# dmosopt/dmosopt

Hardware: NVIDIA H100
Metric: candidate-evals/sec (GP+sort+HV) pop=65536 dim=30 obj=3 (higher is better)
Workload: dtype f64 results; GP variance contraction in split-fp16 wgmma with fp32 accumulation (precision=auto: calibrated against the float64 path, 0 of 65535 rows of the last step recomputed in float64); ranks on u32 ids

## Files before the change

dmosopt_b200/_lib.py:

```python

import ctypes
import os
import threading

import numpy as np

_HERE = os.path.dirname(os.path.abspath(__file__))
LIB_PATH = os.path.join(_HERE, "libdmosopt_b200.so")

METRIC_NONE, METRIC_CROWDING, METRIC_EUCLIDEAN = 0, 1, 2
KERNEL_MATERN52, KERNEL_RBF = 0, 1
GP_FP64, GP_TENSOR, GP_AUTO = 0, 1, 2
HV_MAX_OBJECTIVES = 8

_c_i64 = ctypes.c_int64
_c_u64 = ctypes.c_uint64
_c_int = ctypes.c_int
_c_dbl = ctypes.c_double
_vp = ctypes.c_void_p

_SIGNATURES = {
    "dmo_version": (_c_int, []),
    "dmo_create": (_c_int, [_c_int, ctypes.POINTER(_vp)]),
    "dmo_destroy": (_c_int, [_vp]),
    "dmo_last_error": (ctypes.c_char_p, [_vp]),
    "dmo_synchronize": (_c_int, [_vp]),
    "dmo_stream": (_vp, [_vp]),
    "dmo_launch_count": (_c_i64, [_vp]),
    "dmo_sm_count": (_c_int, [_vp]),
    "dmo_timer_begin": (_c_int, [_vp]),
    "dmo_timer_end": (_c_int, [_vp, ctypes.POINTER(ctypes.c_float)]),
    "dmo_host_alloc": (_c_int, [ctypes.POINTER(_vp), _c_u64]),
    "dmo_host_free": (_c_int, [_vp]),
    "dmo_device_alloc": (_c_int, [_vp, ctypes.POINTER(_vp), _c_u64]),
    "dmo_device_free": (_c_int, [_vp, _vp]),
    "dmo_memcpy": (_c_int, [_vp, _vp, _vp, _c_u64]),
    "dmo_flush_l2": (_c_int, [_vp]),
    "dmo_transfer_bytes": (_c_int, [_vp, ctypes.POINTER(_c_u64), ctypes.POINTER(_c_u64)]),
    "dmo_profile_enable": (_c_int, [_vp, _c_int]),
    "dmo_profile_report": (_c_int, [_vp, ctypes.c_char_p, _c_u64]),
    "dmo_round_f32": (_c_int, [_vp, _vp, _c_i64]),
    "dmo_rank_nd": (_c_int, [_vp, _vp, _c_i64, _c_int, _vp]),
    "dmo_crowding_distance": (_c_int, [_vp, _vp, _c_i64, _c_int, _vp]),
    "dmo_euclidean_distance": (_c_int, [_vp, _vp, _c_i64, _c_int, _vp]),
    "dmo_order_mo": (_c_int, [_vp, _vp, _c_i64, _c_int, _c_int, _vp, _c_int, _vp, _vp, _vp]),
    "dmo_remove_worst": (_c_int, [_vp, _vp, _vp, _c_i64, _c_int, _c_int, _c_int, _vp, _c_int, _c_i64, _vp, _vp, _vp, _vp]),
    "dmo_remove_worst_pair": (_c_int, [_vp, _vp, _vp, _c_i64, _vp, _vp, _c_i64, _c_int, _c_int, _c_int, _c_i64, _vp, _vp, _vp, _vp]),
    "dmo_tournament": (_c_int, [_vp, _vp, _vp, _c_i64, _c_i64, _c_u64, _c_u64, _vp, _vp]),
    "dmo_mutation_u": (_c_int, [_vp, _vp, _vp, _c_i64, _c_int, _vp, _vp, _vp, _c_dbl, _vp]),
    "dmo_sbx_u": (_c_int, [_vp, _vp, _vp, _vp, _c_i64, _c_int, _vp, _vp, _vp, _vp, _vp]),
    "dmo_nsga2_plan_length": (_c_i64, [_c_i64, _c_dbl, _c_dbl]),
    "dmo_nsga2_generate": (
        _c_int,
        [_vp, _vp, _c_i64, _c_int, _vp, _c_i64, _c_i64, _c_dbl, _c_dbl, _c_dbl, _vp, _vp, _vp, _vp, _c_u64, _c_u64, _vp, _vp, _vp, _vp],
    ),
    "dmo_gp_create": (_c_int, [_vp, _c_i64, _c_int, _c_int, _c_int, _vp, _vp, _vp, _c_int, _vp, _vp, _vp, _vp, _vp, _vp, _vp, ctypes.POINTER(_vp)]),
    "dmo_gp_destroy": (_c_int, [_vp, _vp]),
    "dmo_gp_fit": (_c_int, [_vp, _c_i64, _c_int, _c_int, _c_int, _vp, _vp, _vp, _vp, _vp, _c_dbl, _vp, _vp, _vp]),
    "dmo_gp_set_linear_mean": (_c_int, [_vp, _vp, _vp, _vp]),
    "dmo_gp_predict": (_c_int, [_vp, _vp, _vp, _c_i64, _vp, _vp, _c_int]),
    "dmo_gp_auto_info": (_c_int, [_vp, _vp, ctypes.POINTER(_c_int), ctypes.POINTER(_c_int), ctypes.POINTER(_c_dbl), ctypes.POINTER(_c_dbl),
                                  ctypes.POINTER(_c_dbl), ctypes.POINTER(_c_i64)]),
    "dmo_gp_covariance_groups": (_c_int, [_vp, _vp, ctypes.POINTER(_c_int), _vp]),
    "dmo_mtgp_create": (_c_int, [_vp, _c_i64, _c_int, _c_int, _vp, _vp, _vp, _vp, _vp, _vp, _vp, _vp, _vp, _vp, _vp, ctypes.POINTER(_c_dbl),
                                 ctypes.POINTER(_vp)]),
    "dmo_mtgp_predict": (_c_int, [_vp, _vp, _vp, _c_i64, _vp, _vp, _c_int]),
    "dmo_mtgp_destroy": (_c_int, [_vp, _vp]),
    "dmo_svgp_create": (_c_int, [_vp, _c_int, _c_int, _c_i64, _c_int, _vp, _vp, _vp, _vp, _vp, _vp, _c_dbl, _vp, _vp, _vp, _vp, _vp,
                                 ctypes.POINTER(_vp)]),
    "dmo_svgp_predict": (_c_int, [_vp, _vp, _vp, _c_i64, _vp, _vp, _c_int]),
    "dmo_svgp_groups": (_c_int, [_vp, _vp, ctypes.POINTER(_c_int), ctypes.POINTER(_c_int)]),
    "dmo_svgp_destroy": (_c_int, [_vp, _vp]),
    "dmo_svgp_optimal_q": (_c_int, [_vp, _c_i64, _c_i64, _c_int, _c_int, _vp, _vp, _vp, _vp, _vp, _vp, _c_dbl, _c_int, _vp, _vp]),
    "dmo_mtgp_lml_grad": (_c_int, [_vp, _c_i64, _c_int, _c_int, _vp, _vp, _vp, _vp, _vp, _vp, _vp, _vp, _vp, _vp, _vp, _vp, _vp]),
    "dmo_gp_lml_grad": (_c_int, [_vp, _c_i64, _c_int, _c_int, _vp, _vp, _vp, _vp, _vp, _vp, _vp, _vp, _vp, _vp, _vp, _vp, _vp]),
    "dmo_nsga2_step": (_c_int, [_vp, _vp, _vp, _vp, _vp, _c_i64, _c_int, _c_int, _c_dbl, _c_dbl, _c_dbl, _vp, _vp, _vp, _vp, _c_u64, _c_u64,
                                _c_int, _c_int, _c_int, _c_int, _vp, _vp, _vp]),
    "dmo_hypervolume": (_c_int, [_vp, _vp, _c_i64, _c_int, _vp, ctypes.POINTER(_c_dbl)]),
    "dmo_hypervolume_ranked": (_c_int, [_vp, _vp, _c_i64, _c_int, _vp, _vp, ctypes.POINTER(_c_dbl)]),
    "dmo_ehvi_select": (_c_int, [_vp, _vp, _c_i64, _vp, _vp, _c_i64, _c_int, _vp, _c_int, _c_i64, _vp, _vp]),
    "dmo_get_duplicates": (_c_int, [_vp, _vp, _c_i64, _c_int, _c_dbl, _vp]),
    "dmo_get_duplicates_pair": (_c_int, [_vp, _vp, _c_i64, _vp, _c_i64, _c_int, _c_dbl, _vp]),
    "dmo_age_survival": (_c_int, [_vp, _vp, _vp, _c_i64, _c_int, _c_dbl, _vp, _c_int, _vp]),
    "dmo_smpso_velocity": (_c_int, [_vp, _vp, _vp, _vp, _vp, _c_int, _c_i64, _c_int, _c_dbl, _c_dbl, _c_dbl, _c_dbl, _c_dbl, _c_dbl, _vp, _vp, _vp]),
    "dmo_mutate_groups": (_c_int, [_vp, _vp, _c_i64, _c_i64, _c_i64, _c_int, _vp, _vp, _vp, _c_dbl, _c_u64, _c_u64, _vp, _vp]),
    "dmo_cmaes_sample": (_c_int, [_vp, _vp, _vp, _c_int, _vp, _c_i64, _vp, _vp, _c_i64, _c_int, _vp]),
    "dmo_cmaes_update_cholesky": (_c_int, [_vp, _vp, _vp, _vp, _vp, _vp, _c_i64, _c_int, _c_dbl, _c_dbl, _c_dbl]),
    "dmo_gather_rows": (_c_int, [_vp, _vp, _vp, _vp, _vp, _c_i64, _c_i64, _vp]),
    "dmo_cmaes_generate": (_c_int, [_vp, _vp, _vp, _c_int, _vp, _c_i64, _vp, _vp, _c_i64, _c_int, _vp, _vp, _vp]),
    "dmo_cmaes_step_z": (_c_int, [_vp, _vp, _vp, _vp, _vp, _vp, _vp, _vp, _c_i64, _c_int, _vp]),
    "dmo_scale_rows": (_c_int, [_vp, _vp, _c_i64, _c_i64, _vp, _vp, _vp, _c_i64]),
    "dmo_benchmark_eval": (_c_int, [_vp, _c_int, _vp, _c_i64, _c_int, _c_int, _c_dbl, _vp]),
    "dmo_smpso_generate": (_c_int, [_vp, _vp, _vp, _c_int, _c_i64, _c_int, _vp, _vp, _vp, _c_dbl, _c_u64, _c_u64, _vp, _vp]),
    "dmo_smpso_update": (_c_int, [_vp, _vp, _vp, _vp, _vp, _c_int, _vp, _c_int, _c_i64, _c_int, _c_int, _c_int, _vp, _vp, _vp, _vp, _vp, _vp, _vp]),
}

_lib = None
_ctx = None
_ctx_device = None
_lock = threading.Lock()


class DmoError(RuntimeError):
    pass


def load_library(path=None):
    global _lib
    if _lib is not None:
        return _lib
    path = path or LIB_PATH
    if not os.path.exists(path):
        raise DmoError(
            f"dmosopt_b200: CUDA library {path} not found. Build it with `python -m dmosopt_b200.build` "
            "(nvcc, sm_90a). There is no CPU fallback."
        )
# ... 46 lines not shown
    with _lock:
        while len(_worker_ctx) <= i:
            h = _vp()
            st = load_library().dmo_create(_ctx_device, ctypes.byref(h))
            if st != 0 or not h.value:
                raise DmoError(f"dmosopt_b200: dmo_create(device={_ctx_device}) failed for a worker context (status {st})")
            _worker_ctx.append(h)
    assert main is not None
    return _worker_ctx[i]


def worker_pool():
    global _worker_pool
    if _worker_pool is None:
        from concurrent.futures import ThreadPoolExecutor

        _worker_pool = ThreadPoolExecutor(max_workers=8, thread_name_prefix="dmosopt_b200_worker")
    return _worker_pool


def _ptr(a):
    if a is None:
        return None
    if isinstance(a, np.ndarray):
        return a.ctypes.data
    if hasattr(a, "data_ptr"):
        return int(a.data_ptr())
    if isinstance(a, int):
        return a
    raise TypeError(f"cannot pass {type(a)} to the CUDA library")


def _f64(a):
    return np.ascontiguousarray(a, dtype=np.float64)


def synchronize():
    _check(load_library().dmo_synchronize(context()), "dmo_synchronize")


def stream_ptr():
    return int(load_library().dmo_stream(context()))


def launch_count():
    lib = load_library()
    return int(lib.dmo_launch_count(context())) + sum(int(lib.dmo_launch_count(c)) for c in _worker_ctx)


def sm_count():
    return int(load_library().dmo_sm_count(context()))


def timer_begin():
    _check(load_library().dmo_timer_begin(context()), "dmo_timer_begin")


def timer_end():
    ms = ctypes.c_float()
    _check(load_library().dmo_timer_end(context(), ctypes.byref(ms)), "dmo_timer_end")
    return float(ms.value)


def flush_l2():
    _check(load_library().dmo_flush_l2(context()), "dmo_flush_l2")


def transfer_bytes():
    h2d = d2h = 0
    for c in [context()] + list(_worker_ctx):
        a, b = _c_u64(0), _c_u64(0)
        _check(load_library().dmo_transfer_bytes(c, ctypes.byref(a), ctypes.byref(b)), "dmo_transfer_bytes")
        h2d, d2h = h2d + int(a.value), d2h + int(b.value)
    return h2d, d2h


def profile_enable(on=True):
    _check(load_library().dmo_profile_enable(context(), 1 if on else 0), "dmo_profile_enable")


def profile_report():
    buf = ctypes.create_string_buffer(1 << 16)
    _check(load_library().dmo_profile_report(context(), buf, len(buf)), "dmo_profile_report")
    out = {}
    for line in buf.value.decode().splitlines():
        name, ms, cnt = line.rsplit(" ", 2)
        out[name] = (float(ms), int(cnt))
    return out


def round_f32(dev_ptr, n):
    _check(load_library().dmo_round_f32(context(), _ptr(dev_ptr), int(n)), "dmo_round_f32")


class DeviceArray:

    def __init__(self, shape, dtype=np.float64):
        self.shape = tuple(np.atleast_1d(shape).tolist()) if not isinstance(shape, tuple) else shape
        self.dtype = np.dtype(dtype)
        self.nbytes = int(np.prod(self.shape)) * self.dtype.itemsize
        p = _vp()
        _check(load_library().dmo_device_alloc(context(), ctypes.byref(p), max(self.nbytes, 1)), "dmo_device_alloc")
        self.ptr = p.value

    def data_ptr(self):
        return self.ptr
# ... 893 lines not shown
```

dmosopt_b200/csrc/gp_tensor.cu:

```cuda
#include <cuda.h>
#include <cuda_fp16.h>
#include <cudaTypedefs.h>
#include <stdlib.h>

#include "gp.cuh"

namespace {

constexpr int TN = 256;
constexpr int TMV = 128;
constexpr int TK = 32;
constexpr int UK = 16;
constexpr int STAGES = 4;
constexpr int A_BYTES = TMV * TK * 2;
constexpr int B_BYTES = TN * TK * 2;
constexpr int STAGE_BYTES = 2 * A_BYTES + 2 * B_BYTES;
constexpr size_t GEMM_SMEM = (size_t)STAGES * STAGE_BYTES + 1024 + 256;
constexpr int NTHREADS = 384;

__device__ __forceinline__ uint32_t smem_u32(const void* p) { return (uint32_t)__cvta_generic_to_shared(p); }

__device__ __forceinline__ void mbar_init(uint64_t* bar, uint32_t count) {
  asm volatile("mbarrier.init.shared::cta.b64 [%0], %1;" ::"r"(smem_u32(bar)), "r"(count) : "memory");
}
__device__ __forceinline__ void mbar_arrive(uint64_t* bar) {
  asm volatile("mbarrier.arrive.shared::cta.b64 _, [%0];" ::"r"(smem_u32(bar)) : "memory");
}
__device__ __forceinline__ void mbar_expect_tx(uint64_t* bar, uint32_t bytes) {
  asm volatile("mbarrier.arrive.expect_tx.shared::cta.b64 _, [%0], %1;" ::"r"(smem_u32(bar)), "r"(bytes) : "memory");
}
__device__ __forceinline__ bool mbar_try_wait(uint64_t* bar, uint32_t parity) {
  uint32_t ok;
  asm volatile(
      "{\n"
      ".reg .pred p;\n"
      "mbarrier.try_wait.parity.shared::cta.b64 p, [%1], %2;\n"
      "selp.u32 %0, 1, 0, p;\n"
      "}\n"
      : "=r"(ok)
      : "r"(smem_u32(bar)), "r"(parity)
      : "memory");
  return ok != 0;
}
__device__ __forceinline__ void mbar_wait(uint64_t* bar, uint32_t parity, volatile int* abort_flag) {
  uint32_t spins = 0;
  while (!mbar_try_wait(bar, parity)) {
    if ((++spins & 0x3FFu) == 0u) {
      if (*abort_flag) return;
      if (spins > (1u << 22)) {
        *abort_flag = 1;
        return;
      }
    }
  }
}

__device__ __forceinline__ void tma_load_2d(const CUtensorMap* map, uint64_t* bar, void* dst, int c0, int c1) {
  asm volatile(
      "cp.async.bulk.tensor.2d.shared::cluster.global.tile.mbarrier::complete_tx::bytes [%0], [%1, {%3, %4}], [%2];" ::"r"(
          smem_u32(dst)),
      "l"(map), "r"(smem_u32(bar)), "r"(c0), "r"(c1)
      : "memory");
}

__device__ __forceinline__ uint64_t make_sdesc64(uint32_t smem_addr) {
  return (uint64_t)((smem_addr >> 4) & 0x3FFFu) | (1ull << 16) | ((uint64_t)(512 >> 4) << 32) | (2ull << 62);
}

__device__ __forceinline__ void wgmma_fence() { asm volatile("wgmma.fence.sync.aligned;" ::: "memory"); }
__device__ __forceinline__ void wgmma_commit() { asm volatile("wgmma.commit_group.sync.aligned;" ::: "memory"); }
template <int N>
__device__ __forceinline__ void wgmma_wait() {
  asm volatile("wgmma.wait_group.sync.aligned %0;" ::"n"(N) : "memory");
}

__device__ __forceinline__ void wgmma_f16_m64n256(float (&d)[128], uint64_t adesc, uint64_t bdesc, uint32_t accumulate) {
  asm volatile(
      "{\n"
      ".reg .pred p;\n"
      "setp.ne.b32 p, %130, 0;\n"
      "wgmma.mma_async.sync.aligned.m64n256k16.f32.f16.f16 "
      "{"
      "%0, %1, %2, %3, %4, %5, %6, %7, %8, %9, %10, %11, %12, %13, %14, %15, "
      "%16, %17, %18, %19, %20, %21, %22, %23, %24, %25, %26, %27, %28, %29, %30, %31, "
      "%32, %33, %34, %35, %36, %37, %38, %39, %40, %41, %42, %43, %44, %45, %46, %47, "
      "%48, %49, %50, %51, %52, %53, %54, %55, %56, %57, %58, %59, %60, %61, %62, %63, "
      "%64, %65, %66, %67, %68, %69, %70, %71, %72, %73, %74, %75, %76, %77, %78, %79, "
      "%80, %81, %82, %83, %84, %85, %86, %87, %88, %89, %90, %91, %92, %93, %94, %95, "
      "%96, %97, %98, %99, %100, %101, %102, %103, %104, %105, %106, %107, %108, %109, %110, %111, "
      "%112, %113, %114, %115, %116, %117, %118, %119, %120, %121, %122, %123, %124, %125, %126, %127}, "
      "%128, %129, p, 1, 1, 0, 0;\n"
      "}\n"
      : "+f"(d[0]), "+f"(d[1]), "+f"(d[2]), "+f"(d[3]), "+f"(d[4]), "+f"(d[5]), "+f"(d[6]), "+f"(d[7]),
        "+f"(d[8]), "+f"(d[9]), "+f"(d[10]), "+f"(d[11]), "+f"(d[12]), "+f"(d[13]), "+f"(d[14]), "+f"(d[15]),
        "+f"(d[16]), "+f"(d[17]), "+f"(d[18]), "+f"(d[19]), "+f"(d[20]), "+f"(d[21]), "+f"(d[22]), "+f"(d[23]),
        "+f"(d[24]), "+f"(d[25]), "+f"(d[26]), "+f"(d[27]), "+f"(d[28]), "+f"(d[29]), "+f"(d[30]), "+f"(d[31]),
        "+f"(d[32]), "+f"(d[33]), "+f"(d[34]), "+f"(d[35]), "+f"(d[36]), "+f"(d[37]), "+f"(d[38]), "+f"(d[39]),
        "+f"(d[40]), "+f"(d[41]), "+f"(d[42]), "+f"(d[43]), "+f"(d[44]), "+f"(d[45]), "+f"(d[46]), "+f"(d[47]),
        "+f"(d[48]), "+f"(d[49]), "+f"(d[50]), "+f"(d[51]), "+f"(d[52]), "+f"(d[53]), "+f"(d[54]), "+f"(d[55]),
        "+f"(d[56]), "+f"(d[57]), "+f"(d[58]), "+f"(d[59]), "+f"(d[60]), "+f"(d[61]), "+f"(d[62]), "+f"(d[63]),
        "+f"(d[64]), "+f"(d[65]), "+f"(d[66]), "+f"(d[67]), "+f"(d[68]), "+f"(d[69]), "+f"(d[70]), "+f"(d[71]),
        "+f"(d[72]), "+f"(d[73]), "+f"(d[74]), "+f"(d[75]), "+f"(d[76]), "+f"(d[77]), "+f"(d[78]), "+f"(d[79]),
        "+f"(d[80]), "+f"(d[81]), "+f"(d[82]), "+f"(d[83]), "+f"(d[84]), "+f"(d[85]), "+f"(d[86]), "+f"(d[87]),
        "+f"(d[88]), "+f"(d[89]), "+f"(d[90]), "+f"(d[91]), "+f"(d[92]), "+f"(d[93]), "+f"(d[94]), "+f"(d[95]),
        "+f"(d[96]), "+f"(d[97]), "+f"(d[98]), "+f"(d[99]), "+f"(d[100]), "+f"(d[101]), "+f"(d[102]), "+f"(d[103]),
        "+f"(d[104]), "+f"(d[105]), "+f"(d[106]), "+f"(d[107]), "+f"(d[108]), "+f"(d[109]), "+f"(d[110]), "+f"(d[111]),
        "+f"(d[112]), "+f"(d[113]), "+f"(d[114]), "+f"(d[115]), "+f"(d[116]), "+f"(d[117]), "+f"(d[118]), "+f"(d[119]),
        "+f"(d[120]), "+f"(d[121]), "+f"(d[122]), "+f"(d[123]), "+f"(d[124]), "+f"(d[125]), "+f"(d[126]), "+f"(d[127])
      : "l"(adesc), "l"(bdesc), "r"(accumulate)
      : "memory");
}

struct GemmParams {
  int M, n_pb, n_jt, n_q;
  int64_t k_rows, l_rows;
  const float* inv_scale;
  double* vnorm;
  int64_t vn_ld;
  int* abort_flag;
};

__device__ __forceinline__ int item_blocks(const GemmParams& p, int q) { return q == p.n_jt - 1 - q ? 1 : 2; }
__device__ __forceinline__ int item_row_block(const GemmParams& p, int q, int s) { return s ? p.n_jt - 1 - q : q; }

__global__ void __launch_bounds__(NTHREADS, 1)
    gp_var_wgmma_kernel(const __grid_constant__ CUtensorMap map_kh, const __grid_constant__ CUtensorMap map_kl,
                        const __grid_constant__ CUtensorMap map_lh, const __grid_constant__ CUtensorMap map_ll,
                        const GemmParams prm) {
  extern __shared__ uint8_t smem_raw[];
  uint8_t* tiles = (uint8_t*)(((uintptr_t)smem_raw + 1023) & ~(uintptr_t)1023);
  uint64_t* bars = (uint64_t*)(tiles + (size_t)STAGES * STAGE_BYTES);
  uint64_t* full = bars;
  uint64_t* empty = bars + STAGES;
  volatile int* abort_flag = prm.abort_flag;
  const int warp = threadIdx.x >> 5, lane = threadIdx.x & 31;

  if (threadIdx.x == 0) {
    for (int s = 0; s < STAGES; ++s) {
      mbar_init(&full[s], 1);
      mbar_init(&empty[s], 8);
    }
    asm volatile("fence.mbarrier_init.release.cluster;" ::: "memory");
  }
  __syncthreads();
  const int per_m = prm.n_pb * prm.n_q;
  const int n_work = prm.M * per_m;

  if (warp >= 8) {
    asm volatile("setmaxnreg.dec.sync.aligned.u32 40;\n" ::: "memory");
    if (warp == 8 && lane == 0) {
      uint32_t stage = 0, phase = 0;
      for (int w = blockIdx.x; w < n_work; w += gridDim.x) {
        const int m = w / per_m, r = w - m * per_m;
        const int pb = r / prm.n_q, q = r - pb * prm.n_q;
        const int a_row = (int)(m * prm.k_rows + (int64_t)pb * TMV);
        const int nb = item_blocks(prm, q);
        for (int s = 0; s < nb; ++s) {
          const int jt = item_row_block(prm, q, s);
          const int b_row = (int)(m * prm.l_rows + (int64_t)jt * TN);
          const int nkc = (jt + 1) * (TN / TK);
          for (int kc = 0; kc < nkc; ++kc) {
            mbar_wait(&empty[stage], phase ^ 1u, abort_flag);
            uint8_t* st = tiles + (size_t)stage * STAGE_BYTES;
            mbar_expect_tx(&full[stage], STAGE_BYTES);
            tma_load_2d(&map_kh, &full[stage], st, kc * TK, a_row);
            tma_load_2d(&map_kl, &full[stage], st + A_BYTES, kc * TK, a_row);
            tma_load_2d(&map_lh, &full[stage], st + 2 * A_BYTES, kc * TK, b_row);
            tma_load_2d(&map_ll, &full[stage], st + 2 * A_BYTES + B_BYTES, kc * TK, b_row);
            if (++stage == STAGES) {
              stage = 0;
              phase ^= 1u;
            }
          }
        }
      }
    }
    return;
  }

  asm volatile("setmaxnreg.inc.sync.aligned.u32 232;\n" ::: "memory");
  const int wg = warp >> 2;
  const int row0 = wg * 64 + (warp & 3) * 16 + (lane >> 2);
  const int col0 = 2 * (lane & 3);
  float acc[128];
  uint32_t stage = 0, phase = 0;
  for (int w = blockIdx.x; w < n_work; w += gridDim.x) {
    const int m = w / per_m, r = w - m * per_m;
    const int pb = r / prm.n_q, q = r - pb * prm.n_q;
    const float* isc = prm.inv_scale + (int64_t)m * prm.l_rows;
    double total0 = 0.0, total1 = 0.0;
    const int nb = item_blocks(prm, q);
    for (int s = 0; s < nb; ++s) {
      const int jt = item_row_block(prm, q, s);
      const int nkc = (jt + 1) * (TN / TK);
      uint32_t prev = 0;
      for (int kc = 0; kc < nkc; ++kc) {
        mbar_wait(&full[stage], phase, abort_flag);
        const uint32_t sa = smem_u32(tiles + (size_t)stage * STAGE_BYTES);
        const uint32_t a_off = wg * (64 * TK * 2);
        const uint64_t a_hi = make_sdesc64(sa + a_off), a_lo = make_sdesc64(sa + A_BYTES + a_off);
        const uint64_t b_hi = make_sdesc64(sa + 2 * A_BYTES), b_lo = make_sdesc64(sa + 2 * A_BYTES + B_BYTES);
        wgmma_fence();
#pragma unroll
        for (int ks = 0; ks < TK / UK; ++ks) {
          const uint64_t adv = (uint64_t)((ks * UK * 2) >> 4);
          wgmma_f16_m64n256(acc, a_hi + adv, b_hi + adv, (kc | ks) ? 1u : 0u);
          wgmma_f16_m64n256(acc, a_hi + adv, b_lo + adv, 1u);
          wgmma_f16_m64n256(acc, a_lo + adv, b_hi + adv, 1u);
        }
        wgmma_commit();
        if (kc > 0) {
          wgmma_wait<1>();
          if (lane == 0) mbar_arrive(&empty[prev]);
        }
        prev = stage;
        if (++stage == STAGES) {
          stage = 0;
          phase ^= 1u;
        }
      }
      wgmma_wait<0>();
      if (lane == 0) mbar_arrive(&empty[prev]);
      const float* sc = isc + jt * TN + col0;
#pragma unroll
      for (int g = 0; g < TN / 32; ++g) {
        float p0[4] = {0.f, 0.f, 0.f, 0.f}, p1[4] = {0.f, 0.f, 0.f, 0.f};
#pragma unroll
        for (int u = 0; u < 4; ++u) {
          const int i = 4 * g + u;
          const float2 sv = __ldg(reinterpret_cast<const float2*>(sc + 8 * i));
          const float t00 = acc[4 * i] * sv.x, t01 = acc[4 * i + 1] * sv.y;
          const float t10 = acc[4 * i + 2] * sv.x, t11 = acc[4 * i + 3] * sv.y;
          p0[u] = fmaf(t01, t01, t00 * t00);
          p1[u] = fmaf(t11, t11, t10 * t10);
        }
        total0 += ((double)p0[0] + (double)p0[1]) + ((double)p0[2] + (double)p0[3]);
        total1 += ((double)p1[0] + (double)p1[1]) + ((double)p1[2] + (double)p1[3]);
      }
    }
#pragma unroll
    for (int o = 1; o < 4; o <<= 1) {
      total0 += __shfl_xor_sync(0xffffffffu, total0, o);
      total1 += __shfl_xor_sync(0xffffffffu, total1, o);
    }
    if ((lane & 3) == 0) {
      const int64_t o = ((int64_t)q * prm.M + m) * prm.vn_ld + (int64_t)pb * TMV + row0;
      prm.vnorm[o] = total0;
      prm.vnorm[o + 8] = total1;
    }
  }
}

__global__ void split_linv_kernel(const double* __restrict__ Linv, int64_t Npad, const int* __restrict__ k_exp,
                                  uint16_t* __restrict__ Lh, uint16_t* __restrict__ Ll, float* __restrict__ inv_scale) {
  const int64_t row = blockIdx.x;
  const int g = (int)(row / Npad);
  const double* src = Linv + row * Npad;
  __shared__ double red[256];
  double mx = 0.0;
  for (int64_t k = threadIdx.x; k < Npad; k += blockDim.x) mx = fmax(mx, fabs(src[k]));
  red[threadIdx.x] = mx;
  __syncthreads();
  for (int o = 128; o > 0; o >>= 1) {
    if (threadIdx.x < o) red[threadIdx.x] = fmax(red[threadIdx.x], red[threadIdx.x + o]);
    __syncthreads();
  }
  mx = red[0];
  int e = 0;
  if (mx > 0.0) e = 13 - ilogb(mx);
  const double s = scalbn(1.0, e);
  for (int64_t k = threadIdx.x; k < Npad; k += blockDim.x) {
    const float x = (float)(src[k] * s);
    const __half h = __float2half_rn(x);
    const __half l = __float2half_rn(x - __half2float(h));
    Lh[row * Npad + k] = __half_as_ushort(h);
    Ll[row * Npad + k] = __half_as_ushort(l);
  }
  if (threadIdx.x == 0) inv_scale[row] = (mx > 0.0) ? (float)scalbn(1.0, -e - k_exp[g]) : 0.f;
}

constexpr int KT_TN = 128, KT_TP = 32;

__device__ __forceinline__ float stationary_f(float s2, int kind) {
  if (kind == DMO_KERNEL_MATERN52) {
    float r;
    asm("sqrt.approx.ftz.f32 %0, %1;" : "=f"(r) : "f"(s2));
    const float K = r * 2.2360679774997896f;
    return fmaf(K, fmaf(K, 1.0f / 3.0f, 1.0f), 1.0f) * __expf(-K);
  }
  return __expf(-0.5f * s2);
}

__device__ __forceinline__ float2 fadd2(float2 a, float2 b) { return make_float2(__fadd_rn(a.x, b.x), __fadd_rn(a.y, b.y)); }
__device__ __forceinline__ float2 fmul2(float2 a, float2 b) { return make_float2(__fmul_rn(a.x, b.x), __fmul_rn(a.y, b.y)); }
__device__ __forceinline__ float2 ffma2(float2 a, float2 b, float2 c) {
  return make_float2(__fmaf_rn(a.x, b.x, c.x), __fmaf_rn(a.y, b.y, c.y));
}

__device__ __forceinline__ float2 stationary2_f(float2 s2, int kind) {
  float2 e;
  if (kind == DMO_KERNEL_MATERN52) {
    float2 r;
    asm("sqrt.approx.ftz.f32 %0, %1;" : "=f"(r.x) : "f"(s2.x));
// ... 535 lines not shown
      best_eff = eff;
      best = ns;
      *n_per_block = npb;
    }
  }
  return best;
}

int gp_mean_direct(dmo_ctx* ctx, dmo_gp* gp, const double* dXn, int64_t P, double* d_mean) {
  const int64_t N = gp->N, Npad = gp->ops.Npad;
  const int M = gp->M, d = gp->d;
  DMO_TRY(prepare_direct_state(ctx, gp));
  const int64_t n_qb = ceil_div(P, KM_Q);
  int64_t n_per_block = Npad;
  const int64_t nsplit = pick_slices(n_qb, Npad, KM_NS, (int64_t)4 * ctx->sm_count, &n_per_block);
  const int64_t ld = n_qb * KM_Q;
  DevBuf<double> mpart;
  DMO_TRY(mpart.alloc(ctx, (size_t)nsplit * M * ld));
  dim3 grid((unsigned)nsplit, (unsigned)n_qb);
  {
    ProfileScope ps_(ctx, "gp_mean_direct");
#define KM_LAUNCH(ISO_, MT_)                                                                                                  \
  do {                                                                                                                      \
    if (d <= 16)                                                                                                            \
      DMO_LAUNCH((gp_mean_direct_kernel<ISO_, MT_, 4>), grid, KM_T, 0, dXn, P, (int64_t)0, gp->Xtf.p, N, Npad, n_per_block, \
                 d, gp->kernel, gp->inv_ls.p, gp->constant.p, gp->alpha.p, mpart.p, ld);                                    \
    else                                                                                                                    \
      DMO_LAUNCH((gp_mean_direct_kernel<ISO_, MT_, 8>), grid, KM_T, 0, dXn, P, (int64_t)0, gp->Xtf.p, N, Npad, n_per_block, \
                 d, gp->kernel, gp->inv_ls.p, gp->constant.p, gp->alpha.p, mpart.p, ld);                                    \
  } while (0)
#define KM_SWITCH(ISO_)        \
  switch (M) {                 \
    case 1: KM_LAUNCH(ISO_, 1); break; \
    case 2: KM_LAUNCH(ISO_, 2); break; \
    case 3: KM_LAUNCH(ISO_, 3); break; \
    case 4: KM_LAUNCH(ISO_, 4); break; \
    case 5: KM_LAUNCH(ISO_, 5); break; \
    default: KM_LAUNCH(ISO_, 6); break; \
  }
    if (gp->isotropic) {
      KM_SWITCH(true)
    } else {
      KM_SWITCH(false)
    }
#undef KM_SWITCH
#undef KM_LAUNCH
  }
  DMO_LAUNCH(mean_finish_tc_kernel, (unsigned)ceil_div(P * M, 256), 256, 0, mpart.p, (int)nsplit, P, ld, M, gp->ymean.p,
             gp->ystd.p, (int64_t)0, d_mean);
  DMO_CHECK_LAUNCH();
  return DMO_OK;
}

}

int gp_prepare_tensor(dmo_ctx* ctx, GpVarOps& ops) {
  if (ops.tensor_ready) return DMO_OK;
  const int G = ops.G;
  const int64_t Npad = ops.Npad;
  std::vector<int> kexp(G);
  for (int g = 0; g < G; ++g) {
    double c = ops.h_kscale[g];
    kexp[g] = (c > 0.0) ? 13 - ilogb(c) : 13;
  }
  DMO_TRY(ops.Kexp.alloc(ctx, G));
  DMO_CUDA(cudaMemcpyAsync(ops.Kexp.p, kexp.data(), G * sizeof(int), cudaMemcpyHostToDevice, ctx->stream));
  DMO_CUDA(cudaStreamSynchronize(ctx->stream));
  DMO_TRY(ops.Lhi.alloc(ctx, (size_t)G * Npad * Npad));
  DMO_TRY(ops.Llo.alloc(ctx, (size_t)G * Npad * Npad));
  DMO_TRY(ops.Lscale.alloc(ctx, (size_t)G * Npad));
  DMO_LAUNCH(split_linv_kernel, (unsigned)(G * Npad), 256, 0, ops.Linv.p, Npad, ops.Kexp.p, ops.Lhi.p, ops.Llo.p,
             ops.Lscale.p);
  DMO_CHECK_LAUNCH();
  ops.tensor_ready = true;
  return DMO_OK;
}

static_assert(TMV == GP_TC_TILE, "gp.cuh exports the wgmma candidate tile");

int gp_tensor_var_planes(int64_t Npad) { return (int)((Npad / TN + 1) / 2); }

int gp_var_contract_tensor(dmo_ctx* ctx, const GpVarOps& ops, const uint16_t* Kh, const uint16_t* Kl, int64_t k_alloc,
                           int64_t k_rows, int64_t Pcpad, double* vnorm, int64_t vn_ld, int* abort_flag) {
  const int64_t Npad = ops.Npad;
  DMO_REQUIRE(Npad % TN == 0 && Pcpad % TMV == 0, "gp_var_contract_tensor: internal padding error");
  CUtensorMap map_kh, map_kl, map_lh, map_ll;
  DMO_TRY(make_map(ctx, &map_kh, Kh, (uint64_t)k_alloc, (uint64_t)Npad, TMV, TK, CU_TENSOR_MAP_SWIZZLE_64B));
  DMO_TRY(make_map(ctx, &map_kl, Kl, (uint64_t)k_alloc, (uint64_t)Npad, TMV, TK, CU_TENSOR_MAP_SWIZZLE_64B));
  DMO_TRY(make_map(ctx, &map_lh, ops.Lhi.p, (uint64_t)ops.G * Npad, (uint64_t)Npad, TN, TK, CU_TENSOR_MAP_SWIZZLE_64B));
  DMO_TRY(make_map(ctx, &map_ll, ops.Llo.p, (uint64_t)ops.G * Npad, (uint64_t)Npad, TN, TK, CU_TENSOR_MAP_SWIZZLE_64B));
  DMO_CUDA(cudaFuncSetAttribute(gp_var_wgmma_kernel, cudaFuncAttributeMaxDynamicSharedMemorySize, (int)GEMM_SMEM));
  GemmParams prm;
  prm.M = ops.G;
  prm.n_pb = (int)(Pcpad / TMV);
  prm.n_jt = (int)(Npad / TN);
  prm.n_q = gp_tensor_var_planes(Npad);
  prm.k_rows = k_rows;
  prm.l_rows = Npad;
  prm.inv_scale = ops.Lscale.p;
  prm.vnorm = vnorm;
  prm.vn_ld = vn_ld;
  prm.abort_flag = abort_flag;
  const int n_work = prm.M * prm.n_pb * prm.n_q;
  const int grid = n_work < ctx->sm_count ? n_work : ctx->sm_count;
  DMO_LAUNCH(gp_var_wgmma_kernel, grid, NTHREADS, GEMM_SMEM, map_kh, map_kl, map_lh, map_ll, prm);
  return DMO_OK;
}

int gp_predict_tensor(dmo_ctx* ctx, dmo_gp* gp, const double* dXn, int64_t P, double* d_mean, double* d_var) {
  const int64_t N = gp->N, Npad = gp->ops.Npad;
  const int M = gp->M, G = gp->ops.G, d = gp->d;
  DMO_REQUIRE(M <= 16, "gp_predict(tensor): at most 16 objectives per model (got %d)", M);
  DMO_REQUIRE(d <= 64, "gp_predict(tensor): at most 64 input dimensions (got %d); use DMO_GP_FP64", d);
  DMO_REQUIRE(Npad % TN == 0, "gp_predict(tensor): internal padding error");
  if (!d_var && d <= KM_D && M <= 6)
    return gp_mean_direct(ctx, gp, dXn, P, d_mean);
  DMO_TRY(gp_prepare_tensor(ctx, gp->ops));
  constexpr int64_t TMv = KM_Q;
  int64_t Pc_max = ((int64_t)6 << 30) / ((int64_t)G * Npad * 4);
  Pc_max = (Pc_max / TMv) * TMv;
  if (Pc_max < TMv) Pc_max = TMv;
  const int64_t Pc_alloc = P < Pc_max ? ceil_div(P, TMv) * TMv : Pc_max;
  const int n_q = gp_tensor_var_planes(Npad);
  DevBuf<uint16_t> Kh, Kl;
  DevBuf<double> vnorm;
  DevBuf<int> abort_flag;
  DMO_TRY(Kh.alloc(ctx, (size_t)G * Pc_alloc * Npad));
  DMO_TRY(Kl.alloc(ctx, (size_t)G * Pc_alloc * Npad));
  DMO_TRY(vnorm.alloc(ctx, (size_t)n_q * G * Pc_alloc));
  DMO_TRY(abort_flag.alloc(ctx, 1));
  DMO_CUDA(cudaMemsetAsync(abort_flag.p, 0, sizeof(int), ctx->stream));
  const int64_t kplane = Pc_alloc * Npad;
  const bool fused = d <= KM_D && M <= 6 && (gp->isotropic || G <= 2) &&
                     !(getenv("DMO_GP_FUSED") && atoi(getenv("DMO_GP_FUSED")) == 0);
  DevBuf<double> mpart;
  if (fused) DMO_TRY(prepare_direct_state(ctx, gp));
  for (int64_t p_base = 0; p_base < P; p_base += Pc_alloc) {
    const int64_t Pc = (P - p_base) < Pc_alloc ? (P - p_base) : Pc_alloc;
    const int64_t Pcpad = ceil_div(Pc, TMv) * TMv;
    if (fused) {
      int64_t n_per_block = Npad;
      const int64_t n_qb = Pcpad / KM_Q;
      const int64_t nsplit = pick_slices(n_qb, Npad, KF_NS, (int64_t)3 * ctx->sm_count, &n_per_block);
      DMO_TRY(mpart.alloc(ctx, (size_t)nsplit * M * Pcpad));
      dim3 gf((unsigned)nsplit, (unsigned)(Pcpad / KS_Q));
      const size_t smem = kstar_mean_smem(M);
      {
        ProfileScope ps_(ctx, "gp_kstar");
#define KF_LAUNCH(ISO_, MT_, GR_)                                                                                          \
  do {                                                                                                                     \
    DMO_CUDA(cudaFuncSetAttribute(kstar_mean_kernel<ISO_, MT_, GR_>, cudaFuncAttributeMaxDynamicSharedMemorySize, (int)smem)); \
    DMO_LAUNCH((kstar_mean_kernel<ISO_, MT_, GR_>), gf, KS_T, smem, dXn, P, p_base, gp->Xtf.p, N, Npad, n_per_block, d,          \
               gp->kernel, G, gp->cov.p, gp->g_inv_ls.p, gp->g_constant.p, gp->ops.Kexp.p, gp->CAf.p, kplane, Kh.p, Kl.p,   \
               mpart.p, Pcpad);                                                                                            \
  } while (0)
#define KF_SWITCH(ISO_)                                         \
  if (G < M) {                                                  \
// ... 72 lines not shown
```

include/dmosopt_b200.h:

```cpp
#ifndef DMOSOPT_B200_H
#define DMOSOPT_B200_H

#include <stdint.h>

#ifdef __cplusplus
extern "C" {
#endif

#define DMO_OK 0
#define DMO_ERR_CUDA 1
#define DMO_ERR_ARG 2
#define DMO_ERR_STATE 3
#define DMO_ERR_UNSUPPORTED 4
#define DMO_ERR_INTERNAL 5

#define DMO_METRIC_NONE 0
#define DMO_METRIC_CROWDING 1
#define DMO_METRIC_EUCLIDEAN 2

#define DMO_KERNEL_MATERN52 0
#define DMO_KERNEL_RBF 1

#define DMO_GP_FP64 0
#define DMO_GP_TENSOR 1
// ... 32 lines not shown

int dmo_order_mo(dmo_ctx* ctx, const double* Y, int64_t n, int M, int metric,
                 const double* const* extra_desc_keys, int n_extra,
                 int64_t* perm, int32_t* rank_sorted, double* dist_sorted);
int dmo_remove_worst(dmo_ctx* ctx, const double* X, const double* Y, int64_t n, int d, int M,
                     int metric, const double* const* extra_desc_keys, int n_extra, int64_t keep,
                     double* X_out, double* Y_out, int32_t* rank_out, int64_t* perm_out);

int dmo_remove_worst_pair(dmo_ctx* ctx, const double* Xa, const double* Ya, int64_t na, const double* Xb,
                          const double* Yb, int64_t nb, int d, int M, int metric, int64_t keep,
                          double* X_out, double* Y_out, int32_t* rank_out, int64_t* perm_out);

int dmo_tournament(dmo_ctx* ctx, const int32_t* rank, const double* crowd, int64_t pop,
                   int64_t poolsize, uint64_t seed, uint64_t stream_id,
                   int64_t* pool_idx, double* u_out);

int dmo_mutation_u(dmo_ctx* ctx, const double* parents, const double* u, int64_t n, int d,
                   const double* di_mutation, const double* xlb, const double* xub,
                   double mutation_rate, double* children);
int dmo_sbx_u(dmo_ctx* ctx, const double* parent1, const double* parent2, const double* u,
              int64_t n, int d, const double* di_crossover, const double* xlb, const double* xub,
              double* child1, double* child2);

int64_t dmo_nsga2_plan_length(int64_t popsize, double crossover_prob, double mutation_prob);
int dmo_nsga2_generate(dmo_ctx* ctx, const double* pop_x, int64_t npop, int d,
                       const int64_t* pool_idx, int64_t poolsize, int64_t popsize,
                       double crossover_prob, double mutation_prob, double mutation_rate,
                       const double* di_crossover, const double* di_mutation,
                       const double* xlb, const double* xub, uint64_t seed, uint64_t stream_id,
                       double* x_gen, int32_t* child_kind, int64_t* n_children, double* draws);

int dmo_nsga2_step(dmo_ctx* ctx, dmo_gp* gp, double* pop_x, double* pop_y, int32_t* rank, int64_t pop,
                   int d, int M, double crossover_prob, double mutation_prob, double mutation_rate,
                   const double* di_crossover, const double* di_mutation, const double* xlb,
                   const double* xub, uint64_t seed, uint64_t stream_id, int precision,
                   int distance_metric, int with_variance, int round_to_f32, const double* hv_ref,
                   int64_t* n_children, double* hv_out);

int dmo_gp_create(dmo_ctx* ctx, int64_t N, int d, int M, int kernel, const double* X_train,
                  const double* alpha, const double* factor, int factor_is_inverse,
                  const double* constant, const double* length_scale, const double* noise,
                  const double* y_mean, const double* y_std, const double* xlb, const double* xub,
                  dmo_gp** out);
int dmo_gp_destroy(dmo_ctx* ctx, dmo_gp* gp);
int dmo_gp_fit(dmo_ctx* ctx, int64_t N, int d, int M, int kernel, const double* X_train, const double* y,
               const double* constant, const double* length_scale, const double* noise, double jitter,
               double* L_out, double* alpha_out, double* lml_out);
int dmo_gp_set_linear_mean(dmo_ctx* ctx, dmo_gp* gp, const double* weight, const double* bias);
int dmo_gp_predict(dmo_ctx* ctx, dmo_gp* gp, const double* X, int64_t P, double* mean,
                   double* var, int precision);
int dmo_gp_auto_info(dmo_ctx* ctx, dmo_gp* gp, int* mean_tensor, int* var_tensor, double* mean_err,
                     double* var_err, double* theta, int64_t* last_refined);
int dmo_gp_covariance_groups(dmo_ctx* ctx, dmo_gp* gp, int* n_groups, int* group_of);

int dmo_mtgp_create(dmo_ctx* ctx, int64_t N, int d, int M, const double* X_train, const double* Y,
                    const double* length_scale, const double* B, const double* D, const double* weight,
                    const double* bias, const double* y_mean, const double* y_std, const double* xlb,
                    const double* xub, double* lml_out, dmo_mtgp** out);
int dmo_mtgp_predict(dmo_ctx* ctx, dmo_mtgp* mt, const double* X, int64_t P, double* mean, double* var,
                     int precision);
int dmo_mtgp_destroy(dmo_ctx* ctx, dmo_mtgp* mt);
int dmo_mtgp_lml_grad(dmo_ctx* ctx, int64_t N, int d, int M, const double* X_train, const double* Y,
                      const double* length_scale, const double* B, const double* D, const double* weight,
                      const double* bias, double* lml_out, double* g_length_scale, double* g_B, double* g_D,
                      double* g_weight, double* g_bias);
int dmo_gp_lml_grad(dmo_ctx* ctx, int64_t N, int d, int M, const double* X_train, const double* y,
                    const double* length_scale, const double* outputscale, const double* noise, const double* weight,
                    const double* bias, double* lml_out, double* g_length_scale, double* g_outputscale,
                    double* g_noise, double* g_weight, double* g_bias);

int dmo_svgp_create(dmo_ctx* ctx, int L, int M, int64_t Z, int d, const double* Zpts, const double* variance,
                    const double* length_scale, const double* q_mu, const double* q_sqrt, const double* W, double jitter,
                    const double* y_mean, const double* y_std, const double* y_var_scale, const double* xlb,
                    const double* xrng, dmo_svgp** out);
int dmo_svgp_predict(dmo_ctx* ctx, dmo_svgp* sv, const double* X, int64_t P, double* mean, double* var, int precision);
int dmo_svgp_groups(dmo_ctx* ctx, dmo_svgp* sv, int* n_groups, int* n_planes);
int dmo_svgp_destroy(dmo_ctx* ctx, dmo_svgp* sv);
int dmo_svgp_optimal_q(dmo_ctx* ctx, int64_t N, int64_t Z, int d, int L, const double* X, const double* y,
                       const double* Zpts, const double* variance, const double* length_scale, const double* noise,
                       double jitter, int inducing_is_data, double* q_mu_out, double* q_sqrt_out);

int dmo_hypervolume(dmo_ctx* ctx, const double* F, int64_t n, int M, const double* ref, double* out);
int dmo_hypervolume_ranked(dmo_ctx* ctx, const double* F, int64_t n, int M, const double* ref,
                           const int32_t* rank, double* out);

int dmo_ehvi_select(dmo_ctx* ctx, const double* F, int64_t nf, const double* means,
                    const double* variances, int64_t nc, int M, const double* ref, int nds,
                    int64_t k, int64_t* sel, double* score);

int dmo_get_duplicates(dmo_ctx* ctx, const double* X, int64_t n, int d, double eps, uint8_t* is_dup);
int dmo_get_duplicates_pair(dmo_ctx* ctx, const double* X, int64_t n, const double* Y, int64_t ny, int d,
                            double eps, uint8_t* is_dup);

int dmo_age_survival(dmo_ctx* ctx, const double* yn, const double* nn, int64_t m, int M, double p,
                     const int32_t* extreme, int n_ext, double* crowd);

int dmo_smpso_velocity(dmo_ctx* ctx, const float* position, const double* velocity, const double* leader1,
                       const double* leader2, int f32_difference, int64_t n, int d, double w, double c1,
                       double r1, double c2, double r2, double chi, const double* xlb, const double* xub,
                       double* out);
int dmo_mutate_groups(dmo_ctx* ctx, const double* pop_x, int64_t group_size, int64_t n_groups,
                      int64_t per_group, int d, const double* di_mutation, const double* xlb,
                      const double* xub, double mutation_rate, uint64_t seed, uint64_t stream_id,
                      double* children, int64_t* parent_rows);
int dmo_smpso_generate(dmo_ctx* ctx, const double* parm, const double* vel, int swarms, int64_t pop, int d,
                       const double* di_mutation, const double* xlb, const double* xub, double mutation_rate,
// ... 39 lines not shown
```

Before: 6.173 million.

## Share L-factor tiles across 2-CTA clusters via TMA multicast in GP variance GEMM

Launches the wgmma variance contraction kernel as clusters of two CTAs that process adjacent row blocks for the same column tile. Each CTA loads half of the shared B (L inverse hi/lo) tile and multicasts it to both CTAs. Empty-barrier releases are sent cluster-wide so a stage is refilled only after both consumers finish with it. This roughly halves global/L2 traffic for the B operand, at the cost of cross-CTA synchronisation, padding work when the row-block count is odd, and a grid capped by cluster occupancy.

Result: faster. 6.303 million, median of 6 (+2.1%).

```diff
diff --git a/dmosopt_b200/_lib.py b/dmosopt_b200/_lib.py
--- a/dmosopt_b200/_lib.py
+++ b/dmosopt_b200/_lib.py
@@ -62,6 +62,7 @@
     "dmo_gp_auto_info": (_c_int, [_vp, _vp, ctypes.POINTER(_c_int), ctypes.POINTER(_c_int), ctypes.POINTER(_c_dbl), ctypes.POINTER(_c_dbl),
                                   ctypes.POINTER(_c_dbl), ctypes.POINTER(_c_i64)]),
     "dmo_gp_covariance_groups": (_c_int, [_vp, _vp, ctypes.POINTER(_c_int), _vp]),
+    "dmo_gp_var_clusters": (_c_int, [_vp, ctypes.POINTER(_c_int), ctypes.POINTER(_c_int)]),
     "dmo_mtgp_create": (_c_int, [_vp, _c_i64, _c_int, _c_int, _vp, _vp, _vp, _vp, _vp, _vp, _vp, _vp, _vp, _vp, _vp, ctypes.POINTER(_c_dbl),
                                  ctypes.POINTER(_vp)]),
     "dmo_mtgp_predict": (_c_int, [_vp, _vp, _vp, _c_i64, _vp, _vp, _c_int]),
@@ -214,6 +215,12 @@
     return int(load_library().dmo_sm_count(context()))
 
 
+def gp_var_clusters():
+    c, n = _c_int(0), _c_int(0)
+    _check(load_library().dmo_gp_var_clusters(context(), ctypes.byref(c), ctypes.byref(n)), "dmo_gp_var_clusters")
+    return c.value, n.value
+
+
 def timer_begin():
     _check(load_library().dmo_timer_begin(context()), "dmo_timer_begin")
 
diff --git a/dmosopt_b200/csrc/gp_tensor.cu b/dmosopt_b200/csrc/gp_tensor.cu
--- a/dmosopt_b200/csrc/gp_tensor.cu
+++ b/dmosopt_b200/csrc/gp_tensor.cu
@@ -12,6 +12,8 @@
 constexpr int TK = 32;
 constexpr int UK = 16;
 constexpr int STAGES = 4;
+constexpr int CL = 2;
+constexpr int B_SHARE = TN / CL;
 constexpr int A_BYTES = TMV * TK * 2;
 constexpr int B_BYTES = TN * TK * 2;
 constexpr int STAGE_BYTES = 2 * A_BYTES + 2 * B_BYTES;
@@ -23,11 +25,18 @@
 __device__ __forceinline__ void mbar_init(uint64_t* bar, uint32_t count) {
   asm volatile("mbarrier.init.shared::cta.b64 [%0], %1;" ::"r"(smem_u32(bar)), "r"(count) : "memory");
 }
-__device__ __forceinline__ void mbar_arrive(uint64_t* bar) {
-  asm volatile("mbarrier.arrive.shared::cta.b64 _, [%0];" ::"r"(smem_u32(bar)) : "memory");
-}
 __device__ __forceinline__ void mbar_expect_tx(uint64_t* bar, uint32_t bytes) {
   asm volatile("mbarrier.arrive.expect_tx.shared::cta.b64 _, [%0], %1;" ::"r"(smem_u32(bar)), "r"(bytes) : "memory");
+}
+__device__ __forceinline__ void mbar_arrive_cluster(uint64_t* bar, uint32_t rank) {
+  asm volatile(
+      "{\n"
+      ".reg .b32 ra;\n"
+      "mapa.shared::cluster.u32 ra, %0, %1;\n"
+      "mbarrier.arrive.shared::cluster.b64 _, [ra];\n"
+      "}\n" ::"r"(smem_u32(bar)),
+      "r"(rank)
+      : "memory");
 }
 __device__ __forceinline__ bool mbar_try_wait(uint64_t* bar, uint32_t parity) {
   uint32_t ok;
@@ -61,6 +70,23 @@
           smem_u32(dst)),
       "l"(map), "r"(smem_u32(bar)), "r"(c0), "r"(c1)
       : "memory");
+}
+__device__ __forceinline__ void tma_load_2d_multicast(const CUtensorMap* map, uint64_t* bar, void* dst, int c0, int c1,
+                                                      uint16_t mask) {
+  asm volatile(
+      "cp.async.bulk.tensor.2d.shared::cluster.global.tile.mbarrier::complete_tx::bytes.multicast::cluster"
+      " [%0], [%1, {%4, %5}], [%2], %3;" ::"r"(smem_u32(dst)),
+      "l"(map), "r"(smem_u32(bar)), "h"(mask), "r"(c0), "r"(c1)
+      : "memory");
+}
+
+__device__ __forceinline__ uint32_t cluster_ctarank() {
+  uint32_t r;
+  asm volatile("mov.u32 %0, %%cluster_ctarank;" : "=r"(r));
+  return r;
+}
+__device__ __forceinline__ void cluster_sync() {
+  asm volatile("barrier.cluster.arrive.release.aligned;\nbarrier.cluster.wait.acquire.aligned;" ::: "memory");
 }
 
 __device__ __forceinline__ uint64_t make_sdesc64(uint32_t smem_addr) {
@@ -123,7 +149,7 @@
 __device__ __forceinline__ int item_blocks(const GemmParams& p, int q) { return q == p.n_jt - 1 - q ? 1 : 2; }
 __device__ __forceinline__ int item_row_block(const GemmParams& p, int q, int s) { return s ? p.n_jt - 1 - q : q; }
 
-__global__ void __launch_bounds__(NTHREADS, 1)
+__global__ void __cluster_dims__(CL, 1, 1) __launch_bounds__(NTHREADS, 1)
     gp_var_wgmma_kernel(const __grid_constant__ CUtensorMap map_kh, const __grid_constant__ CUtensorMap map_kl,
                         const __grid_constant__ CUtensorMap map_lh, const __grid_constant__ CUtensorMap map_ll,
                         const GemmParams prm) {
@@ -134,39 +160,45 @@
   uint64_t* empty = bars + STAGES;
   volatile int* abort_flag = prm.abort_flag;
   const int warp = threadIdx.x >> 5, lane = threadIdx.x & 31;
+  const int crank = (int)cluster_ctarank();
+  const int cluster = blockIdx.x / CL, n_clusters = gridDim.x / CL;
 
   if (threadIdx.x == 0) {
     for (int s = 0; s < STAGES; ++s) {
       mbar_init(&full[s], 1);
-      mbar_init(&empty[s], 8);
+      mbar_init(&empty[s], 8 * CL);
     }
     asm volatile("fence.mbarrier_init.release.cluster;" ::: "memory");
   }
-  __syncthreads();
-  const int per_m = prm.n_pb * prm.n_q;
+  cluster_sync();
+  const int n_grp = (prm.n_pb + CL - 1) / CL;
+  const int per_m = n_grp * prm.n_q;
   const int n_work = prm.M * per_m;
 
   if (warp >= 8) {
     asm volatile("setmaxnreg.dec.sync.aligned.u32 40;\n" ::: "memory");
     if (warp == 8 && lane == 0) {
+      const uint16_t mask = (uint16_t)((1u << CL) - 1u);
       uint32_t stage = 0, phase = 0;
-      for (int w = blockIdx.x; w < n_work; w += gridDim.x) {
+      for (int w = cluster; w < n_work; w += n_clusters) {
         const int m = w / per_m, r = w - m * per_m;
-        const int pb = r / prm.n_q, q = r - pb * prm.n_q;
+        const int grp = r / prm.n_q, q = r - grp * prm.n_q;
+        const int pb = min(grp * CL + crank, prm.n_pb - 1);
         const int a_row = (int)(m * prm.k_rows + (int64_t)pb * TMV);
         const int nb = item_blocks(prm, q);
         for (int s = 0; s < nb; ++s) {
           const int jt = item_row_block(prm, q, s);
-          const int b_row = (int)(m * prm.l_rows + (int64_t)jt * TN);
+          const int b_row = (int)(m * prm.l_rows + (int64_t)jt * TN) + crank * B_SHARE;
           const int nkc = (jt + 1) * (TN / TK);
           for (int kc = 0; kc < nkc; ++kc) {
             mbar_wait(&empty[stage], phase ^ 1u, abort_flag);
             uint8_t* st = tiles + (size_t)stage * STAGE_BYTES;
+            uint8_t* sb = st + 2 * A_BYTES + crank * (B_SHARE * TK * 2);
             mbar_expect_tx(&full[stage], STAGE_BYTES);
             tma_load_2d(&map_kh, &full[stage], st, kc * TK, a_row);
             tma_load_2d(&map_kl, &full[stage], st + A_BYTES, kc * TK, a_row);
-            tma_load_2d(&map_lh, &full[stage], st + 2 * A_BYTES, kc * TK, b_row);
-            tma_load_2d(&map_ll, &full[stage], st + 2 * A_BYTES + B_BYTES, kc * TK, b_row);
+            tma_load_2d_multicast(&map_lh, &full[stage], sb, kc * TK, b_row, mask);
+            tma_load_2d_multicast(&map_ll, &full[stage], sb + B_BYTES, kc * TK, b_row, mask);
             if (++stage == STAGES) {
               stage = 0;
               phase ^= 1u;
@@ -175,6 +207,8 @@
         }
       }
     }
+    __syncwarp();
+    cluster_sync();
     return;
   }
 
@@ -182,11 +216,17 @@
   const int wg = warp >> 2;
   const int row0 = wg * 64 + (warp & 3) * 16 + (lane >> 2);
   const int col0 = 2 * (lane & 3);
+  auto release = [&](uint32_t slot) {
+    if (lane == 0)
+#pragma unroll
+      for (int c = 0; c < CL; ++c) mbar_arrive_cluster(&empty[slot], (uint32_t)c);
+  };
   float acc[128];
   uint32_t stage = 0, phase = 0;
-  for (int w = blockIdx.x; w < n_work; w += gridDim.x) {
+  for (int w = cluster; w < n_work; w += n_clusters) {
     const int m = w / per_m, r = w - m * per_m;
-    const int pb = r / prm.n_q, q = r - pb * prm.n_q;
+    const int grp = r / prm.n_q, q = r - grp * prm.n_q;
+    const int pb = grp * CL + crank;
     const float* isc = prm.inv_scale + (int64_t)m * prm.l_rows;
     double total0 = 0.0, total1 = 0.0;
     const int nb = item_blocks(prm, q);
@@ -211,7 +251,7 @@
         wgmma_commit();
         if (kc > 0) {
           wgmma_wait<1>();
-          if (lane == 0) mbar_arrive(&empty[prev]);
+          release(prev);
         }
         prev = stage;
         if (++stage == STAGES) {
@@ -220,7 +260,7 @@
         }
       }
       wgmma_wait<0>();
-      if (lane == 0) mbar_arrive(&empty[prev]);
+      release(prev);
       const float* sc = isc + jt * TN + col0;
 #pragma unroll
       for (int g = 0; g < TN / 32; ++g) {
@@ -243,12 +283,13 @@
       total0 += __shfl_xor_sync(0xffffffffu, total0, o);
       total1 += __shfl_xor_sync(0xffffffffu, total1, o);
     }
-    if ((lane & 3) == 0) {
+    if ((lane & 3) == 0 && pb < prm.n_pb) {
       const int64_t o = ((int64_t)q * prm.M + m) * prm.vn_ld + (int64_t)pb * TMV + row0;
       prm.vnorm[o] = total0;
       prm.vnorm[o + 8] = total1;
     }
   }
+  cluster_sync();
 }
 
 __global__ void split_linv_kernel(const double* __restrict__ Linv, int64_t Npad, const int* __restrict__ k_exp,
@@ -890,6 +931,31 @@
   return DMO_OK;
 }
 
+int gp_var_max_clusters(dmo_ctx* ctx) {
+  static int cache[64] = {0};
+  const int dev = ctx->device;
+  if (dev >= 0 && dev < 64 && cache[dev] > 0) return cache[dev];
+  if (cudaFuncSetAttribute(gp_var_wgmma_kernel, cudaFuncAttributeMaxDynamicSharedMemorySize, (int)GEMM_SMEM) != cudaSuccess)
+    return 0;
+  cudaLaunchConfig_t cfg = {};
+  cfg.gridDim = dim3(CL * (unsigned)ctx->sm_count, 1, 1);
+  cfg.blockDim = dim3(NTHREADS, 1, 1);
+  cfg.dynamicSmemBytes = GEMM_SMEM;
+  cfg.stream = ctx->stream;
+  int n = 0;
+  if (cudaOccupancyMaxActiveClusters(&n, gp_var_wgmma_kernel, &cfg) != cudaSuccess) return 0;
+  if (dev >= 0 && dev < 64) cache[dev] = n;
+  return n;
+}
+
+}
+
+extern "C" int dmo_gp_var_clusters(dmo_ctx* ctx, int* cluster_size, int* active_clusters) {
+  const int n = gp_var_max_clusters(ctx);
+  if (n < 1) return dmo_fail(ctx, DMO_ERR_CUDA, "dmo_gp_var_clusters: occupancy query for clusters of %d CTAs failed", CL);
+  if (cluster_size) *cluster_size = CL;
+  if (active_clusters) *active_clusters = n;
+  return DMO_OK;
 }
 
 int gp_prepare_tensor(dmo_ctx* ctx, GpVarOps& ops) {
@@ -925,9 +991,11 @@
   CUtensorMap map_kh, map_kl, map_lh, map_ll;
   DMO_TRY(make_map(ctx, &map_kh, Kh, (uint64_t)k_alloc, (uint64_t)Npad, TMV, TK, CU_TENSOR_MAP_SWIZZLE_64B));
   DMO_TRY(make_map(ctx, &map_kl, Kl, (uint64_t)k_alloc, (uint64_t)Npad, TMV, TK, CU_TENSOR_MAP_SWIZZLE_64B));
-  DMO_TRY(make_map(ctx, &map_lh, ops.Lhi.p, (uint64_t)ops.G * Npad, (uint64_t)Npad, TN, TK, CU_TENSOR_MAP_SWIZZLE_64B));
-  DMO_TRY(make_map(ctx, &map_ll, ops.Llo.p, (uint64_t)ops.G * Npad, (uint64_t)Npad, TN, TK, CU_TENSOR_MAP_SWIZZLE_64B));
+  DMO_TRY(make_map(ctx, &map_lh, ops.Lhi.p, (uint64_t)ops.G * Npad, (uint64_t)Npad, B_SHARE, TK, CU_TENSOR_MAP_SWIZZLE_64B));
+  DMO_TRY(make_map(ctx, &map_ll, ops.Llo.p, (uint64_t)ops.G * Npad, (uint64_t)Npad, B_SHARE, TK, CU_TENSOR_MAP_SWIZZLE_64B));
   DMO_CUDA(cudaFuncSetAttribute(gp_var_wgmma_kernel, cudaFuncAttributeMaxDynamicSharedMemorySize, (int)GEMM_SMEM));
+  const int max_clusters = gp_var_max_clusters(ctx);
+  if (max_clusters < 1) return dmo_fail(ctx, DMO_ERR_CUDA, "gp_var_contract_tensor: no cluster of %d CTAs fits on the device", CL);
   GemmParams prm;
   prm.M = ops.G;
   prm.n_pb = (int)(Pcpad / TMV);
@@ -939,8 +1007,8 @@
   prm.vnorm = vnorm;
   prm.vn_ld = vn_ld;
   prm.abort_flag = abort_flag;
-  const int n_work = prm.M * prm.n_pb * prm.n_q;
-  const int grid = n_work < ctx->sm_count ? n_work : ctx->sm_count;
+  const int n_work = prm.M * (int)ceil_div(prm.n_pb, CL) * prm.n_q;
+  const int grid = CL * (n_work < max_clusters ? n_work : max_clusters);
   DMO_LAUNCH(gp_var_wgmma_kernel, grid, NTHREADS, GEMM_SMEM, map_kh, map_kl, map_lh, map_ll, prm);
   return DMO_OK;
 }
diff --git a/include/dmosopt_b200.h b/include/dmosopt_b200.h
--- a/include/dmosopt_b200.h
+++ b/include/dmosopt_b200.h
@@ -108,6 +108,7 @@
 int dmo_gp_auto_info(dmo_ctx* ctx, dmo_gp* gp, int* mean_tensor, int* var_tensor, double* mean_err,
                      double* var_err, double* theta, int64_t* last_refined);
 int dmo_gp_covariance_groups(dmo_ctx* ctx, dmo_gp* gp, int* n_groups, int* group_of);
+int dmo_gp_var_clusters(dmo_ctx* ctx, int* cluster_size, int* active_clusters);
 
 int dmo_mtgp_create(dmo_ctx* ctx, int64_t N, int d, int M, const double* X_train, const double* Y,
                     const double* length_scale, const double* B, const double* D, const double* weight,
```
